# bruAristimunha/Synthetic-Sleep-EEG-Signal-Generation-using-Latent-Diffusion-Models

Hardware: AMD Instinct MI355X
Metric: EEG windows/sec (LDM train step) (higher is better)
Workload: dtype bf16; 1 GPU; LDM train step on raw (B,1,3072) windows: frozen AutoencoderKL[32,32,64] encode+sample x scale, add_noise, config_ldm.yaml UNet (30.5M params, latent_channels=1) fwd+bwd, epsilon MSE, Adam lr 1e-4 [BASELINE configs[2]/[3]: per-GPU batch 256 = global 2048 / 8]; per_gpu_batch=256, global_batch=256, latent_len=768, parallelism=dp1

## Files before the change

### synthetic-sleep-eeg-signal-generation-using-latent-diffusion-models_amd/csrc/norm.hip

```cpp
#include "common.h"
#include "internal.h"
#include <stdlib.h>

namespace {

constexpr int NT = 256;
constexpr int MAXG_LDS = 1024;
constexpr int GN_NSLOT = 64;
constexpr int GN_FOLD_MAX = 96;
constexpr size_t GN_REGION_FLOATS = (size_t)GN_NSLOT * 2 * 1024;
constexpr size_t GN_SLOT_OFFSET = 1u << 20;
constexpr size_t GN_SLOT_OFFSET_B = (1u << 20) + (512u << 10);
constexpr size_t GN_SLOT_OFFSET_C[2] = {24u << 20, (24u << 20) + (512u << 10)};
static inline size_t gn_slot_region(int region) { return region == 0 ? GN_SLOT_OFFSET_B : GN_SLOT_OFFSET_C[(region - 1) & 1]; }

template <typename T, int V> struct Vec;
template <> struct Vec<float, 4> { typedef float4 type; };
template <> struct Vec<bf16_t, 4> { typedef uint2 type; };
template <> struct Vec<f16_t, 4> { typedef uint2 type; };

template <typename T> __device__ __forceinline__ void load4(const T* p, float v[4]);
template <> __device__ __forceinline__ void load4<float>(const float* p, float v[4]) {
  float4 t = *(const float4*)p; v[0] = t.x; v[1] = t.y; v[2] = t.z; v[3] = t.w;
}
template <> __device__ __forceinline__ void load4<bf16_t>(const bf16_t* p, float v[4]) {
  uint2 t = *(const uint2*)p;
  v[0] = __uint_as_float(t.x << 16); v[1] = __uint_as_float(t.x & 0xffff0000u);
  v[2] = __uint_as_float(t.y << 16); v[3] = __uint_as_float(t.y & 0xffff0000u);
}
template <> __device__ __forceinline__ void load4<f16_t>(const f16_t* p, float v[4]) {
  uint2 t = *(const uint2*)p;
  v[0] = w16_lo<f16_t>(t.x); v[1] = w16_hi<f16_t>(t.x); v[2] = w16_lo<f16_t>(t.y); v[3] = w16_hi<f16_t>(t.y);
}
template <typename T> __device__ __forceinline__ void unpack4(const typename Vec<T, 4>::type& t, float v[4]);
template <> __device__ __forceinline__ void unpack4<f16_t>(const uint2& t, float v[4]) {
  v[0] = w16_lo<f16_t>(t.x); v[1] = w16_hi<f16_t>(t.x); v[2] = w16_lo<f16_t>(t.y); v[3] = w16_hi<f16_t>(t.y);
}
template <> __device__ __forceinline__ void unpack4<float>(const float4& t, float v[4]) { v[0] = t.x; v[1] = t.y; v[2] = t.z; v[3] = t.w; }
template <> __device__ __forceinline__ void unpack4<bf16_t>(const uint2& t, float v[4]) {
  v[0] = __uint_as_float(t.x << 16); v[1] = __uint_as_float(t.x & 0xffff0000u);
  v[2] = __uint_as_float(t.y << 16); v[3] = __uint_as_float(t.y & 0xffff0000u);
}
template <typename T> __device__ __forceinline__ void store4(T* p, const float v[4]);
template <> __device__ __forceinline__ void store4<float>(float* p, const float v[4]) {
  *(float4*)p = make_float4(v[0], v[1], v[2], v[3]);
}
template <> __device__ __forceinline__ void store4<bf16_t>(bf16_t* p, const float v[4]) {
  uint2 t;
  t.x = pack_bf16x2(v[0], v[1]);
  t.y = pack_bf16x2(v[2], v[3]);
  *(uint2*)p = t;
}
template <> __device__ __forceinline__ void store4<f16_t>(f16_t* p, const float v[4]) {
  uint2 t; t.x = pack_f16x2(v[0], v[1]); t.y = pack_f16x2(v[2], v[3]); *(uint2*)p = t;
}
template <typename T, int V> __device__ __forceinline__ void loadv(const T* p, float v[V]) {
  if constexpr (V == 4) load4<T>(p, v); else v[0] = ld_f32(p);
}
template <typename T, int V> __device__ __forceinline__ void storev(T* p, const float v[V]) {
  if constexpr (V == 4) store4<T>(p, v); else st_f32(p, v[0]);
}

template <typename T> __device__ __forceinline__ double gn_inv_n(int cpg, int L) {
  if constexpr (sizeof(T) == 2) return 1.0 / ((double)cpg * (double)L);
  else return (double)(1.0f / ((float)cpg * (float)L));
}
template <typename T> __device__ __forceinline__ float gn_split_group_mean(double sum, double inv_n) {
  if constexpr (sizeof(T) == 2) return (float)(sum * inv_n);
  else return (float)sum * (float)inv_n;
}

struct ColMap { int TX, TY, ncols; };
__device__ __forceinline__ ColMap colmap(int C, int V) {
  ColMap m; m.ncols = C / V;
  if (m.ncols >= NT) { m.TX = NT; m.TY = 1; } else { m.TX = m.ncols; m.TY = NT / m.ncols; }
  return m;
}

template <typename T, int V>
__global__ __launch_bounds__(NT) void gn_stats_kernel(const T* __restrict__ x, long ldx, double* __restrict__ sums,
                                                      int L, int C, int G, int rows_per_block) {
  __shared__ double acc[2 * MAXG_LDS];
  const int b = blockIdx.y, tid = threadIdx.x;
  const int cpg = C / G;
  for (int i = tid; i < 2 * G; i += NT) acc[i] = 0.0;
// ... 186 lines not shown
template <typename T, int V, int RS>
__global__ __launch_bounds__(NT) void gn_bwd_apply_kernel(const T* __restrict__ x, long ldx, const float* __restrict__ gamma,
                                                          const float* __restrict__ beta, const float* __restrict__ stats,
                                                          const T* __restrict__ dy, long lddy, const double* __restrict__ gsums,
                                                          T* __restrict__ dx, long lddx, const T* __restrict__ dxr, long lddxr,
                                                          int L, int C, int G, int silu, int rows_per_block) {
  const int b = blockIdx.y, tid = threadIdx.x, cpg = C / G;
  const ColMap cm = colmap(C, V);
  if (tid >= cm.TX * cm.TY) return;
  const int tx = tid % cm.TX, ty = tid / cm.TX;
  const double inv_n = gn_inv_n<T>(cpg, L);
  const int l0 = blockIdx.x * rows_per_block, l1 = min(L, l0 + rows_per_block);
  for (int col = tx; col < cm.ncols; col += cm.TX) {
    const int c = col * V, g = c / cpg;
    const float mean = stats[((long)b * G + g) * 2], rstd = stats[((long)b * G + g) * 2 + 1];
    const float m1 = gn_split_group_mean<T>(gsums[((long)b * G + g) * 2], inv_n), m2 = gn_split_group_mean<T>(gsums[((long)b * G + g) * 2 + 1], inv_n);
    float ga[V], be[V];
#pragma unroll
    for (int k = 0; k < V; k++) { ga[k] = gamma[c + k]; be[k] = beta[c + k]; }
#pragma unroll 2
    for (int l = l0 + ty; l < l1; l += cm.TY) {
      const long row = (long)b * L + l;
      float v[V], d[V], o[V];
      loadv<T, V>(x + row * ldx + c, v);
      load_dy_eff_c<T, V, RS>(dy, lddy, b, l, L, c, d);
#pragma unroll
      for (int k = 0; k < V; k++) {
        const float xh = (v[k] - mean) * rstd;
        float dz = d[k];
        if (silu) dz *= silu_grad_f(ga[k] * xh + be[k]);
        o[k] = rstd * (dz * ga[k] - m1 - xh * m2);
      }
      if (dxr) {
        float e[V];
        load_dy_eff_c<T, V, RS>(dxr, lddxr, b, l, L, c, e);
#pragma unroll
        for (int k = 0; k < V; k++) o[k] += e[k];
      }
      storev<T, V>(dx + row * lddx + c, o);
    }
  }
}

template <typename T>
__device__ __forceinline__ void load_dy_eff32(const char* base, unsigned ldb, unsigned cb, int l, int resample, float d[4]) {
  if (resample == 0) {
    load4<T>((const T*)(base + ((unsigned)l * ldb + cb)), d);
  } else if (resample == 1) {
    load4<T>((const T*)(base + ((unsigned)(l >> 1) * ldb + cb)), d);
#pragma unroll
    for (int k = 0; k < 4; k++) d[k] *= 0.5f;
  } else {
    float e[4];
    load4<T>((const T*)(base + ((unsigned)(2 * l) * ldb + cb)), d);
    load4<T>((const T*)(base + ((unsigned)(2 * l + 1) * ldb + cb)), e);
#pragma unroll
    for (int k = 0; k < 4; k++) d[k] += e[k];
  }
}
__device__ __forceinline__ long dy_rows(int L, int resample) { return resample == 1 ? L / 2 : (resample == 2 ? 2L * L : L); }

constexpr int NTB = 1024;
constexpr int RES_MAXG = 64;
constexpr int RES_MAXC = 256;

struct ResMap { int TX, TY, tx, ty, c, gl, b; bool act; };
template <int NTH>
__device__ __forceinline__ ResMap resmap(int CC, int C, int cpg, int xcd) {
  ResMap m; m.TX = CC / 4; m.TY = NTH / m.TX;
  const int tid = threadIdx.x;
  const int nchunk = C / CC, lin = blockIdx.x;
  int chunk, b;
  if (xcd) { const int x = lin & 7, j = lin >> 3; b = (j / nchunk) * 8 + x; chunk = j % nchunk; }
  else { chunk = lin % nchunk; b = lin / nchunk; }
  m.b = b;
  m.tx = tid % m.TX; m.ty = tid / m.TX;
  m.c = chunk * CC + m.tx * 4; m.gl = (m.tx * 4) / cpg;
  m.act = tid < m.TX * m.TY && m.c < C;
  return m;
}
__device__ __forceinline__ int res_row(int k, int ty, int TY, bool pair) {
  return pair ? 2 * ((k >> 1) * TY + ty) + (k & 1) : k * TY + ty;
}

#ifdef EEG_STAGE_TIMING
__device__ unsigned long long gn_tlog[4096 * 8];
#define GN_TSTAMP(k) do { if (threadIdx.x == 0) { asm volatile("s_waitcnt vmcnt(0) lgkmcnt(0)" ::: "memory"); gn_tlog[((size_t)blockIdx.y * gridDim.x + blockIdx.x) % 4096 * 8 + (k)] = __builtin_readcyclecounter(); } } while (0)
#else
#define GN_TSTAMP(k) do {} while (0)
#endif
template <typename T, int RPT, int NTH>
__global__ __launch_bounds__(NTH) void gn_fwd_resident_kernel(const T* __restrict__ x, long ldx, const float* __restrict__ gamma,
                                                              const float* __restrict__ beta, T* __restrict__ y, long ldy,
                                                              T* __restrict__ xr, long ldxr, float* __restrict__ stats,
                                                              int L, int C, int G, float eps, int silu, int resample, int CC, int xcd) {
  __shared__ double red[2 * RES_MAXG];
  GN_TSTAMP(0);
  const int cpg = C / G;
  const ResMap m = resmap<NTH>(CC, C, cpg, xcd);
  const int b = m.b;
  const bool pair = resample == 1;
  for (int i = threadIdx.x; i < 2 * RES_MAXG; i += NTH) red[i] = 0.0;
  typename Vec<T, 4>::type raw[RPT];
  const T* xb = x + (long)b * L * ldx + m.c;
  float pv = 0.f;
  if constexpr (sizeof(T) == 2) { if (m.act) pv = ld_f32<T>(x + (long)b * L * ldx + (m.c / cpg) * cpg); }
  if (m.act) {
#pragma unroll
    for (int k = 0; k < RPT; k++) {
      const int l = res_row(k, m.ty, m.TY, pair);
      if (l < L) raw[k] = *(const typename Vec<T, 4>::type*)(xb + (long)l * ldx);
    }
  }
  GN_TSTAMP(1);
  __syncthreads();
  GN_TSTAMP(2);
  const double inv_n = gn_inv_n<T>(cpg, L);
  float mean = 0.f, rstd = 0.f;
  if constexpr (sizeof(T) == 2) {
    float s1 = 0.f, s2 = 0.f;
    if (m.act) {
#pragma unroll
      for (int k = 0; k < RPT; k++) {
        if (res_row(k, m.ty, m.TY, pair) < L) {
          float v[4]; unpack4<T>(raw[k], v);
#pragma unroll
          for (int j = 0; j < 4; j++) v[j] -= pv;
          s1 += (v[0] + v[1]) + (v[2] + v[3]);
          s2 = fmaf(v[0], v[0], s2); s2 = fmaf(v[1], v[1], s2); s2 = fmaf(v[2], v[2], s2); s2 = fmaf(v[3], v[3], s2);
        }
      }
      atomicAdd(&red[m.gl], (double)s1); atomicAdd(&red[RES_MAXG + m.gl], (double)s2);
    }
    __syncthreads();
    GN_TSTAMP(3);
    GN_TSTAMP(4);
    if (!m.act) return;
    const double md = red[m.gl] * inv_n;
    double var = red[RES_MAXG + m.gl] * inv_n - md * md; if (var < 0.0) var = 0.0;
    mean = (float)((double)pv + md);
    rstd = rsqrtf((float)var + eps);
  } else {
  float s = 0.f;
  if (m.act) {
#pragma unroll
    for (int k = 0; k < RPT; k++) {
      if (res_row(k, m.ty, m.TY, pair) < L) { float v[4]; unpack4<T>(raw[k], v); s += (v[0] + v[1]) + (v[2] + v[3]); }
    }
    atomicAdd(&red[m.gl], (double)s);
  }
  __syncthreads();
  GN_TSTAMP(3);
  if (m.act) {
    mean = (float)(red[m.gl] * inv_n);
    float q = 0.f;
#pragma unroll
    for (int k = 0; k < RPT; k++) {
      if (res_row(k, m.ty, m.TY, pair) < L) {
        float v[4]; unpack4<T>(raw[k], v);
#pragma unroll
        for (int j = 0; j < 4; j++) { const float d = v[j] - mean; q += d * d; }
      }
    }
    atomicAdd(&red[RES_MAXG + m.gl], (double)q);
  }
  __syncthreads();
// ... 164 lines not shown
      const unsigned ldb = (unsigned)lddxr * (unsigned)sizeof(T);
#pragma unroll
      for (int k = 0; k < RPT; k++) { const int l = k * m.TY + m.ty, lc = l < L ? l : L - 1; er[k] = *(const typename Vec<T, 4>::type*)(q + ((unsigned)lc * ldb + cb)); }
    }
  }
  __syncthreads();
#ifdef EEG_GN_BWD_NO_LDS_ATOMICS
  if (m.act && m.ty == 0 && (m.tx * 4) % cpg == 0) {
    double p1 = 0.0, p2 = 0.0;
    for (int i = 0; i < cpg; i++) { const double g = (double)gamma[m.c + i]; p1 += g * redc[RES_MAXC + m.tx * 4 + i]; p2 += g * redc[m.tx * 4 + i]; }
    redg[2 * m.gl] = p1; redg[2 * m.gl + 1] = p2;
  }
#else
  if (m.act && m.ty == 0) {
    double p1 = 0.0, p2 = 0.0;
#pragma unroll
    for (int j = 0; j < 4; j++) { p1 += (double)ga[j] * redc[RES_MAXC + m.tx * 4 + j]; p2 += (double)ga[j] * redc[m.tx * 4 + j]; }
    atomicAdd(&redg[2 * m.gl], p1); atomicAdd(&redg[2 * m.gl + 1], p2);
  }
#endif
  GN_TSTAMP(3);
  __syncthreads();
  GN_TSTAMP(4);
  if (m.act) {
    const double inv_n = gn_inv_n<T>(cpg, L);
    const float m1 = (float)(redg[2 * m.gl] * inv_n), m2 = (float)(redg[2 * m.gl + 1] * inv_n);
    if (slots && m.ty == 0) {
      float* sl = slots + (size_t)(b % nslot) * 2 * C;
#pragma unroll
      for (int j = 0; j < 4; j++) { atomicAdd(&sl[m.c + j], (float)redc[m.tx * 4 + j]); atomicAdd(&sl[C + m.c + j], (float)redc[RES_MAXC + m.tx * 4 + j]); }
    }
    const float rm1 = rstd * m1, rm2 = rstd * m2;
    float gr[4];
#pragma unroll
    for (int j = 0; j < 4; j++) gr[j] = ga[j] * rstd;
    float cs[4] = {0.f, 0.f, 0.f, 0.f};
    char* dxs = (char*)(dx + (long)b * L * lddx);
    const char* dxrs = dxr ? (const char*)(dxr + (long)b * dy_rows(L, resample) * lddxr) : nullptr;
    const unsigned lddxb = (unsigned)lddx * (unsigned)sizeof(T), lddxrb = (unsigned)lddxr * (unsigned)sizeof(T);
    const char* dxr2s = dxr2 ? (const char*)(dxr2 + (long)b * L * lddxr2) : nullptr;
    const unsigned lddxr2b = (unsigned)lddxr2 * (unsigned)sizeof(T);
#pragma unroll
    for (int k = 0; k < RPT; k++) {
      const int l = k * m.TY + m.ty;
      if (l < L) {
        float v[4], o[4]; unpack4<T>(raw[k], v);
#pragma unroll
        for (int j = 0; j < 4; j++) {
          const float xh = fmaf(v[j], rstd, -mean * rstd);
          o[j] = fmaf(d[k][j], gr[j], fmaf(xh, -rm2, -rm1));
        }
        if (dxr) {
          float e[4];
          if constexpr (RAW0) unpack4<T>(er[k], e); else load_dy_eff32<T>(dxrs, lddxrb, cb, l, resample, e);
#pragma unroll
          for (int j = 0; j < 4; j++) o[j] += e[j];
        }
        if (dxr2) {
          float e[4];
          load4<T>((const T*)(dxr2s + ((unsigned)l * lddxr2b + cb)), e);
#pragma unroll
          for (int j = 0; j < 4; j++) o[j] += e[j];
        }
#pragma unroll
        for (int j = 0; j < 4; j++) cs[j] += o[j];
        store4<T>((T*)(dxs + ((unsigned)l * lddxb + cb)), o);
      }
    }
    if (colsum_ps) {
#pragma unroll
      for (int j = 0; j < 4; j++) atomicAdd(&redc[2 * RES_MAXC + m.tx * 4 + j], (double)cs[j]);
    }
  }
  GN_TSTAMP(5);
  if (colsum_ps) {
    __syncthreads();
    if (m.act && m.ty == 0) {
#pragma unroll
      for (int j = 0; j < 4; j++) colsum_ps[(long)b * ldps + m.c + j] = (float)redc[2 * RES_MAXC + m.tx * 4 + j];
    }
  }
}

constexpr int PIPE_RPT = 6;
constexpr int PIPE_SLAB = PIPE_RPT * NTB * 8;
constexpr int PIPE_OFF_ST = 3 * PIPE_SLAB;
constexpr int PIPE_OFF_RED = PIPE_OFF_ST + 1024;
constexpr int PIPE_LDS = PIPE_OFF_RED + (2 * RES_MAXG + 3 * RES_MAXC) * 8;

__device__ __forceinline__ void pipe_dma(const void* base, unsigned voff, unsigned lds_off) {
  const unsigned long long u = (unsigned long long)base;
  const unsigned lo = __builtin_amdgcn_readfirstlane((unsigned)u), hi = __builtin_amdgcn_readfirstlane((unsigned)(u >> 32));
  const unsigned long long b = ((unsigned long long)hi << 32) | lo;
  asm volatile("s_mov_b32 m0, %0\n\ts_nop 0\n\tglobal_load_lds_dwordx4 %1, %2" ::"s"(__builtin_amdgcn_readfirstlane(lds_off)), "v"(voff), "s"(b) : "memory", "m0");
}
#define PIPE_BARRIER() asm volatile("s_waitcnt lgkmcnt(0)\n\ts_barrier" ::: "memory")
#ifdef EEG_STAGE_TIMING
#define PIPE_TSTAMP(k, i) do { if (threadIdx.x == 0 && (k) < 8) gn_tlog[(size_t)(blockIdx.x % 512) * 64 + (k) * 8 + (i)] = __builtin_readcyclecounter(); } while (0)
#else
#define PIPE_TSTAMP(k, i) do {} while (0)
#endif

template <bool SILU, bool HAS_ER, typename T16 = bf16_t>
__global__ __launch_bounds__(NTB) void gn_bwd_pipe_kernel(const bf16_t* __restrict__ x, long ldx, const float* __restrict__ gamma,
                                                          const float* __restrict__ beta, const float* __restrict__ stats,
                                                          const bf16_t* __restrict__ dy, long lddy, bf16_t* __restrict__ dx, long lddx,
                                                          const bf16_t* __restrict__ dxr, long lddxr, float* __restrict__ slots,
                                                          float* __restrict__ colsum_ps, long ldps, int B, int L, int C, int G, int CC, int ndg) {
  extern __shared__ __attribute__((aligned(16))) char psm[];
  typedef __attribute__((address_space(3))) void* lds_ptr_t;
  double* const redg = (double*)(psm + PIPE_OFF_RED);
  double* const redc = redg + 2 * RES_MAXG;
  const int tid = threadIdx.x, lane = tid & 63;
  const unsigned wave_u = __builtin_amdgcn_readfirstlane((unsigned)(tid >> 6));
  const unsigned lds0 = (unsigned)(size_t)(lds_ptr_t)psm;
  const int cpg = C / G, nchunk = C / CC;
  const int TX = CC >> 2, TY = NTB / TX;
  const int tx = tid % TX, ty = tid / TX;
  const int xc = blockIdx.x & 7, mb = blockIdx.x >> 3, MB = gridDim.x >> 3;
  const int chunk = mb % nchunk, slot = mb / nchunk, nslot = MB / nchunk;
  const int c = chunk * CC + tx * 4, gl = (tx * 4) / cpg;
  const int noct = B >> 3;
  const int nk = slot < noct ? (noct - slot + nslot - 1) / nslot : 0;
  float ga[4], gl2[4], bl2[4];
#pragma unroll
  for (int j = 0; j < 4; j++) { ga[j] = gamma[c + j]; gl2[j] = ga[j] * 1.4426950408889634f; bl2[j] = beta[c + j] * 1.4426950408889634f; }
  for (int i = tid; i < 2 * RES_MAXG + 3 * RES_MAXC; i += NTB) redg[i] = 0.0;
  asm volatile("" :: "v"(ga[0]), "v"(ga[1]), "v"(ga[2]), "v"(ga[3]), "v"(bl2[0]), "v"(bl2[1]), "v"(bl2[2]), "v"(bl2[3]));
  const int LPR = CC >> 3;
  const int drow = (int)(wave_u * 64 + lane) / LPR, dcol = lane % LPR;
  const unsigned vx = (unsigned)drow * (unsigned)ldx * 2u + (unsigned)dcol * 16u, sx = (unsigned)(1024 / LPR) * (unsigned)ldx * 2u;
  const unsigned vd = (unsigned)drow * (unsigned)lddy * 2u + (unsigned)dcol * 16u, sd = (unsigned)(1024 / LPR) * (unsigned)lddy * 2u;
  const unsigned ve = (unsigned)drow * (unsigned)lddxr * 2u + (unsigned)dcol * 16u, se = (unsigned)(1024 / LPR) * (unsigned)lddxr * 2u;
  const unsigned st_bytes = (unsigned)B * (unsigned)G * 8u;
  const unsigned st_sub = ((unsigned)(chunk * (CC / cpg)) * 8u) & 15u;
  auto issue_xd = [&](int b) __attribute__((always_inline)) {
    const char* xs = (const char*)(x + (long)b * L * ldx + chunk * CC);
    const char* ds = (const char*)(dy + (long)b * L * lddy + chunk * CC);
#pragma unroll
    for (int i = 0; i < 3; i++) pipe_dma(xs, vx + i * sx, lds0 + (unsigned)(i * 16 + wave_u) * 1024u);
#pragma unroll
    for (int i = 0; i < 3; i++) pipe_dma(ds, vd + i * sd, lds0 + PIPE_SLAB + (unsigned)(i * 16 + wave_u) * 1024u);
    {
      const unsigned a0 = (((unsigned)b * (unsigned)G + (unsigned)(chunk * (CC / cpg))) * 8u) & ~15u;
      unsigned a = a0 + (unsigned)lane * 16u; if (a > st_bytes - 16u) a = st_bytes - 16u;
      pipe_dma(stats, a, lds0 + PIPE_OFF_ST);
    }
  };
  auto issue_e = [&](int b) __attribute__((always_inline)) {
    const char* es = (const char*)(dxr + (long)b * L * lddxr + chunk * CC);
#pragma unroll
    for (int i = 0; i < 3; i++) pipe_dma(es, ve + i * se, lds0 + 2 * PIPE_SLAB + (unsigned)(i * 16 + wave_u) * 1024u);
  };
  if (nk > 0) { issue_xd(slot * 8 + xc); if constexpr (HAS_ER) issue_e(slot * 8 + xc); }
  const double inv_n = gn_inv_n<T16>(cpg, L);
  const unsigned rowb = (unsigned)CC * 2u;
  const unsigned lrd0 = (unsigned)ty * rowb + (unsigned)tx * 8u, lrds = (unsigned)TY * rowb;
  const unsigned lddxb = (unsigned)lddx * 2u;
  const unsigned st0 = (unsigned)ty * lddxb + (unsigned)c * 2u, sts = (unsigned)TY * lddxb;
  asm volatile("s_waitcnt vmcnt(0)" ::: "memory");
  for (int k = 0; k < nk; k++) {
    const int b = (slot + k * nslot) * 8 + xc;
    PIPE_TSTAMP(k, 0);
    PIPE_BARRIER();
    PIPE_TSTAMP(k, 1);
    uint2 raw[PIPE_RPT], dr[PIPE_RPT];
// ... 36 lines not shown
      double p1 = 0.0, p2 = 0.0;
#pragma unroll
      for (int j = 0; j < 4; j++) { p1 += (double)ga[j] * redc[RES_MAXC + tx * 4 + j]; p2 += (double)ga[j] * redc[tx * 4 + j]; }
      atomicAdd(&redg[2 * gl], p1); atomicAdd(&redg[2 * gl + 1], p2);
    }
    if constexpr (HAS_ER) {
      if (k + 1 < nk) asm volatile("s_waitcnt vmcnt(7)" ::: "memory"); else asm volatile("s_waitcnt vmcnt(0)" ::: "memory");
    }
    PIPE_BARRIER();
    PIPE_TSTAMP(k, 5);
    {
      const float m1 = (float)(redg[2 * gl] * inv_n), m2 = (float)(redg[2 * gl + 1] * inv_n);
      if (slots && ty == 0) {
        float* sl = slots + (size_t)(b % ndg) * 2 * C;
#pragma unroll
        for (int j = 0; j < 4; j++) { atomicAdd(&sl[c + j], (float)redc[tx * 4 + j]); atomicAdd(&sl[C + c + j], (float)redc[RES_MAXC + tx * 4 + j]); }
      }
      const float rm1 = rstd * m1, rm2 = rstd * m2;
      const float a2 = -rm2 * rstd, b2 = fmaf(-rm2, nmr, -rm1);
      float gr[4];
#pragma unroll
      for (int j = 0; j < 4; j++) gr[j] = ga[j] * rstd;
      float cs[4] = {0.f, 0.f, 0.f, 0.f};
      char* dxs = (char*)(dx + (long)b * L * lddx);
#pragma unroll
      for (int r = 0; r < PIPE_RPT; r++) {
        float v[4], o[4]; unpack4<T16>(raw[r], v);
#pragma unroll
        for (int j = 0; j < 4; j++) o[j] = fmaf(d[r][j], gr[j], fmaf(v[j], a2, b2));
        if constexpr (HAS_ER) {
          float e[4]; unpack4<T16>(*(const uint2*)(psm + 2 * PIPE_SLAB + lrd0 + (unsigned)r * lrds), e);
#pragma unroll
          for (int j = 0; j < 4; j++) o[j] += e[j];
        }
        if (colsum_ps) {
#pragma unroll
          for (int j = 0; j < 4; j++) cs[j] += o[j];
        }
        store4<T16>((T16*)(dxs + (st0 + (unsigned)r * sts)), o);
      }
      if (colsum_ps) {
#pragma unroll
        for (int j = 0; j < 4; j++) atomicAdd(&redc[2 * RES_MAXC + tx * 4 + j], (double)cs[j]);
      }
    }
    PIPE_TSTAMP(k, 6);
    PIPE_BARRIER();
    if (ty == 0) {
#pragma unroll
      for (int j = 0; j < 4; j++) {
        if (colsum_ps) colsum_ps[(long)b * ldps + c + j] = (float)redc[2 * RES_MAXC + tx * 4 + j];
        redc[tx * 4 + j] = 0.0; redc[RES_MAXC + tx * 4 + j] = 0.0; redc[2 * RES_MAXC + tx * 4 + j] = 0.0;
      }
    }
    if (tid < 2 * RES_MAXG) redg[tid] = 0.0;
    if (k + 1 < nk) {
      if constexpr (HAS_ER) { issue_e((slot + (k + 1) * nslot) * 8 + xc); asm volatile("s_waitcnt vmcnt(9)" ::: "memory"); }
      else asm volatile("s_waitcnt vmcnt(6)" ::: "memory");
    }
    PIPE_TSTAMP(k, 7);
  }
}


struct GnRoute { int family, vec, nth, rpt, cc, xcd; };
static thread_local GnRoute g_gn_route[2] = {{0, 0, 0, 0, 0, 0}, {0, 0, 0, 0, 0, 0}};
inline void gn_note(int bwd, int family, int vec, int nth, int rpt, int cc, int xcd) { g_gn_route[bwd] = GnRoute{family, vec, nth, rpt, cc, xcd}; }

int resident_chunk(int L, int C, int G, int resample_pair, int rpt_max, int* rpt_out, int nth = NTB) {
  const int cpg = C / G;
  if (C % 4 != 0 || cpg % 4 != 0) return 0;
  int best = 0, best_rpt = 0;
  for (int mlt = 1; mlt * cpg <= RES_MAXC && mlt <= RES_MAXG; mlt++) {
    const int cc = mlt * cpg;
    if (C % cc != 0) continue;
    const int tx = cc / 4, ty = nth / tx;
    if (ty < 1) break;
    int rpt = resample_pair ? 2 * ((L / 2 + ty - 1) / ty) : (L + ty - 1) / ty;
    if (rpt > rpt_max) break;
    best = cc; best_rpt = rpt;
  }
  *rpt_out = best_rpt;
  return best;
}

int grid_for(long total_threads, eegldm_ctx* ctx) {
  long blocks = (total_threads + NT - 1) / NT;
  long cap = (long)ctx->num_cu * 16;
  return (int)(blocks < cap ? (blocks < 1 ? 1 : blocks) : cap);
}

int pick_lsplit(int B, int L, int C, eegldm_ctx* ctx, int* rows_per_block, int per_cu = 8, int min_rows = 16) {
  int want = (ctx->num_cu * per_cu + B - 1) / B;
  int maxsplit = (L + min_rows - 1) / min_rows;
  int ls = want < 1 ? 1 : (want > maxsplit ? maxsplit : want);
  int rpb = (L + ls - 1) / ls;
  *rows_per_block = rpb;
  return (L + rpb - 1) / rpb;
}

template <typename T, int V>
int gn_fwd_t(eegldm_ctx* ctx, const void* x, long ldx, const float* gamma, const float* beta, void* y, long ldy,
             float* stats, int B, int L, int C, int G, float eps, int silu, int resample, void* xr, long ldxr) {
  if constexpr (V == 4) {
    EEG_ENV_VAR(bool, off, getenv("EEGLDM_GN_NO_RESIDENT") != nullptr);
    constexpr int fwd_rpt_max = 12;
    EEG_ENV_VAR(int, fwd_nth, getenv("EEGLDM_GN_FWD_NTH") ? atoi(getenv("EEGLDM_GN_FWD_NTH")) : 1024);
    int nth = (fwd_nth == 512 || fwd_nth == 256) ? fwd_nth : 1024;
    int rpt = 0; int cc = off ? 0 : resident_chunk(L, C, G, resample == 1, fwd_rpt_max, &rpt, nth);
    EEG_ENV_VAR(bool, no_few, getenv("EEGLDM_GN_NO_FEW_SLAB_NARROW") != nullptr);
    if (!no_few && cc && nth == 1024 && (long)(C / cc) * B <= ctx->num_cu / 4) {
      int rpt2 = 0; const int cc2 = resident_chunk(L, C, G, resample == 1, fwd_rpt_max, &rpt2, 256);
      if (cc2 && cc2 * (int)sizeof(T) >= 32) { nth = 256; cc = cc2; rpt = rpt2; }
    }
    constexpr long fwd_bpc = 4;
    constexpr bool no_xcd = false;
    constexpr int narrow_min = 32;
    const bool can_xcd = !no_xcd && B % 8 == 0;
    const int min_row = nth == 1024 ? (can_xcd ? narrow_min : 128) : 32;
    if (cc && (cc * (int)sizeof(T) < min_row || (long)(C / cc) * B > fwd_bpc * ctx->num_cu * (1024 / nth))) cc = 0;
    if (cc) {
      const int xcd = ((nth < 1024 || cc * (int)sizeof(T) < 128) && can_xcd) ? 1 : 0;
      const dim3 grid((unsigned)((long)(C / cc) * B));
#define GN_FWD_RES1(R, N) hipLaunchKernelGGL((gn_fwd_resident_kernel<T, R, N>), grid, dim3(N), 0, ctx->stream, (const T*)x, ldx, gamma, beta, \
                                         (T*)y, ldy, (T*)xr, ldxr, stats, L, C, G, eps, silu, resample, cc, xcd)
#define GN_FWD_RES(R) do { if (nth == 1024) GN_FWD_RES1(R, 1024); else if (nth == 512) GN_FWD_RES1(R, 512); else GN_FWD_RES1(R, 256); } while (0)
      gn_note(0, 2, 1, nth, rpt <= 6 ? 6 : 12, cc, xcd);
      if (rpt <= 6) GN_FWD_RES(6); else GN_FWD_RES(12);
#undef GN_FWD_RES
#undef GN_FWD_RES1
      LAUNCH_CHECK();
      return 0;
    }
  }
  double* sums = (double*)ctx->scratch;
  int rpb; int ls = pick_lsplit(B, L, C, ctx, &rpb);
  gn_note(0, 1, V == 4, NT, 0, 0, 0);
  hipLaunchKernelGGL((gn_stats_kernel<T, V>), dim3(ls, B), dim3(NT), 0, ctx->stream, (const T*)x, ldx, sums, L, C, G, rpb);
  LAUNCH_CHECK();
  hipLaunchKernelGGL(gn_finalize_kernel, dim3((B * G + 255) / 256), dim3(256), 0, ctx->stream, sums, stats, B * G,
                     (double)(C / G) * (double)L, eps);
  LAUNCH_CHECK();
  int rpb2; int ls2 = pick_lsplit(B, resample == 1 ? L / 2 : L, C, ctx, &rpb2, 16, 8);
  hipLaunchKernelGGL((gn_apply_kernel<T, V>), dim3(ls2, B), dim3(NT), 0, ctx->stream, (const T*)x, ldx, gamma,
                     beta, stats, (T*)y, ldy, (T*)xr, ldxr, L, C, G, silu, resample, rpb2);
  LAUNCH_CHECK();
  return 0;
}

template <typename T, int V>
int gn_bwd_t(eegldm_ctx* ctx, const void* x, long ldx, const float* gamma, const float* beta, const float* stats,
             const void* dy, long lddy, void* dx, long lddx, float* dgamma, float* dbeta, int B, int L, int C, int G,
             int silu, int resample, const void* dxr, long lddxr, float* colsum_ps, long ldps, int* colsum_done,
             const void* dxr2, long lddxr2, int* dxr2_done, int* slots_deferred, int defer_region) {
  if (colsum_done) *colsum_done = 0;
  if (dxr2_done) *dxr2_done = 0;
  if (slots_deferred) *slots_deferred = 0;
  if (!dxr2_done || lddxr2 % 4 != 0) dxr2 = nullptr;
  if constexpr (V == 4) {
    EEG_ENV_VAR(bool, off, getenv("EEGLDM_GN_NO_RESIDENT") != nullptr);
    EEG_ENV_VAR(int, bwd_nth, getenv("EEGLDM_GN_BWD_NTH") ? atoi(getenv("EEGLDM_GN_BWD_NTH")) : 1024);
    EEG_ENV_VAR(bool, unfenced, getenv("EEGLDM_GN_NARROW_UNFENCED") != nullptr);
#ifdef EEG_GN_NO_FENCE
    const int nth = (bwd_nth == 512 || bwd_nth == 256) ? bwd_nth : 1024;
#else
    const int nth = ((bwd_nth == 512 || bwd_nth == 256) && (unfenced || (!ctx->side_on && g_eeg_live_ctx <= 1))) ? bwd_nth : 1024;
// ... 22 lines not shown
          if (dgamma) slots = (float*)((char*)ctx->scratch + (defer ? gn_slot_region(defer_region) : GN_SLOT_OFFSET));
          if (det) {
            ndg = B;
            EEG_TRY(eeg_det_buffer(ctx, (size_t)ndg * 2 * C * sizeof(float), &slots));
            HIP_TRY(hipMemsetAsync(slots, 0, (size_t)ndg * 2 * C * sizeof(float), ctx->stream));
          }
          constexpr bool no_batch_p = false;
          const bool batched = defer && ctx->defer_wgrad && !no_batch_p && C <= 1024 && ctx->gn_fold_count < GN_FOLD_MAX;
          if (batched) {
            if (!ctx->gn_slot_arena) {
              HIP_TRY(hipMalloc(&ctx->gn_slot_arena, (size_t)GN_FOLD_MAX * GN_REGION_FLOATS * sizeof(float)));
              HIP_TRY(hipMemsetAsync(ctx->gn_slot_arena, 0, (size_t)GN_FOLD_MAX * GN_REGION_FLOATS * sizeof(float), ctx->stream));
            }
            slots = ctx->gn_slot_arena + (size_t)ctx->gn_fold_count * GN_REGION_FLOATS;
            ctx->gn_fold_pending.push_back({slots, dgamma, dbeta, C});
            ctx->gn_fold_count++;
          }
          static DevOnce attr_once;
          if (attr_once.need(ctx->device)) {
            HIP_TRY(hipFuncSetAttribute((const void*)gn_bwd_pipe_kernel<true, true, T>, hipFuncAttributeMaxDynamicSharedMemorySize, PIPE_LDS));
            HIP_TRY(hipFuncSetAttribute((const void*)gn_bwd_pipe_kernel<true, false, T>, hipFuncAttributeMaxDynamicSharedMemorySize, PIPE_LDS));
            HIP_TRY(hipFuncSetAttribute((const void*)gn_bwd_pipe_kernel<false, true, T>, hipFuncAttributeMaxDynamicSharedMemorySize, PIPE_LDS));
            HIP_TRY(hipFuncSetAttribute((const void*)gn_bwd_pipe_kernel<false, false, T>, hipFuncAttributeMaxDynamicSharedMemorySize, PIPE_LDS));
          }
          const dim3 grid((unsigned)(8 * nslot * nchunk));
          gn_note(1, 3, 1, NTB, PIPE_RPT, pcc, 1);
#define GN_BWD_PIPE(SL, ER) hipLaunchKernelGGL((gn_bwd_pipe_kernel<SL, ER, T>), grid, dim3(NTB), PIPE_LDS, ctx->stream, (const bf16_t*)x, ldx, gamma, beta, stats, \
                                           (const bf16_t*)dy, lddy, (bf16_t*)dx, lddx, (const bf16_t*)dxr, lddxr, slots, colsum_ps, ldps, B, L, C, G, pcc, ndg)
          if (silu) { if (dxr) GN_BWD_PIPE(true, true); else GN_BWD_PIPE(true, false); }
          else { if (dxr) GN_BWD_PIPE(false, true); else GN_BWD_PIPE(false, false); }
#undef GN_BWD_PIPE
          LAUNCH_CHECK();
          if (det) {
            EEG_TRY(ew_fold_partials_det(ctx, slots, ndg, 2 * C, 0, C, dgamma)); EEG_TRY(ew_fold_partials_det(ctx, slots, ndg, 2 * C, C, C, dbeta));
          } else if (slots && !defer) {
            hipLaunchKernelGGL(gn_slot_reduce_kernel, dim3((2 * C + 255) / 256), dim3(256), 0, ctx->stream, slots, dgamma, dbeta, C, (double*)ctx->scratch, 0, ndg);
            LAUNCH_CHECK();
          }
          if (defer) *slots_deferred = batched ? 2 : 1;
          if (colsum_done && colsum_ps) *colsum_done = 1;
          return 0;
        }
      }
    }
    int rpt = 0; int cc = off ? 0 : resident_chunk(L, C, G, 0, sizeof(T) == 2 ? 12 : 8, &rpt, nth);
    constexpr long bwd_bpc = 8;
    constexpr int bwd_minrow = 128, narrow_min = 32;
    constexpr bool no_xcd = false;
    const bool can_xcd = !no_xcd && B % 8 == 0;
    const int min_row = nth == 1024 ? (can_xcd && narrow_min < bwd_minrow ? narrow_min : bwd_minrow) : 32;
    if (cc && (cc * (int)sizeof(T) < min_row || (long)(C / cc) * B > bwd_bpc * ctx->num_cu * (1024 / nth))) cc = 0;
    if (cc) {
      const int xcd = ((nth < 1024 || cc * (int)sizeof(T) < 128) && can_xcd) ? 1 : 0;
      const dim3 grid((unsigned)((long)(C / cc) * B));
      constexpr bool no_defer = false;
      const bool det = eeg_deterministic() && dgamma;
      const bool defer = slots_deferred && dgamma && !no_defer && !det;
      float* slots = dgamma ? (float*)((char*)ctx->scratch + (defer ? gn_slot_region(defer_region) : GN_SLOT_OFFSET)) : nullptr;
      int nslot = GN_NSLOT;
      if (det) {
        nslot = B;
        EEG_TRY(eeg_det_buffer(ctx, (size_t)nslot * 2 * C * sizeof(float), &slots));
        HIP_TRY(hipMemsetAsync(slots, 0, (size_t)nslot * 2 * C * sizeof(float), ctx->stream));
      }
      constexpr bool no_batch = false;
      const bool batched = defer && ctx->defer_wgrad && !no_batch && C <= 1024 && ctx->gn_fold_count < GN_FOLD_MAX;
      if (batched) {
        if (!ctx->gn_slot_arena) {
          HIP_TRY(hipMalloc(&ctx->gn_slot_arena, (size_t)GN_FOLD_MAX * GN_REGION_FLOATS * sizeof(float)));
          HIP_TRY(hipMemsetAsync(ctx->gn_slot_arena, 0, (size_t)GN_FOLD_MAX * GN_REGION_FLOATS * sizeof(float), ctx->stream));
        }
        slots = ctx->gn_slot_arena + (size_t)ctx->gn_fold_count * GN_REGION_FLOATS;
        ctx->gn_fold_pending.push_back({slots, dgamma, dbeta, C});
        ctx->gn_fold_count++;
      }
#define GN_BWD_RES3(R, RAW, SL, N) hipLaunchKernelGGL((gn_bwd_resident_kernel<T, R, RAW, SL, N>), grid, dim3(N), 0, ctx->stream, (const T*)x, ldx, gamma, beta, stats, \
                                         (const T*)dy, lddy, (T*)dx, lddx, (const T*)dxr, lddxr, slots, colsum_ps, ldps, L, C, G, silu, resample, cc, (const T*)dxr2, lddxr2, xcd, nslot)
#define GN_BWD_RES2(R, RAW, SL) do { if (nth == 1024) GN_BWD_RES3(R, RAW, SL, 1024); else if (nth == 512) GN_BWD_RES3(R, RAW, SL, 512); else GN_BWD_RES3(R, RAW, SL, 256); } while (0)
      constexpr bool raw0 = true;
#define GN_BWD_RES1(R, RAW) do { if (silu) GN_BWD_RES2(R, RAW, true); else GN_BWD_RES2(R, RAW, false); } while (0)
#define GN_BWD_RES(R) do { if (resample == 0 && raw0) GN_BWD_RES1(R, true); else GN_BWD_RES1(R, false); } while (0)
      constexpr int RLO = sizeof(T) == 2 ? 6 : 4, RHI = sizeof(T) == 2 ? 12 : 8;
      gn_note(1, 2, 1, nth, rpt <= RLO ? RLO : RHI, cc, xcd);
      if (rpt <= RLO) GN_BWD_RES(RLO); else GN_BWD_RES(RHI);
#undef GN_BWD_RES
#undef GN_BWD_RES1
#undef GN_BWD_RES2
#undef GN_BWD_RES3
      LAUNCH_CHECK();
      if (det) {
        EEG_TRY(ew_fold_partials_det(ctx, slots, nslot, 2 * C, 0, C, dgamma)); EEG_TRY(ew_fold_partials_det(ctx, slots, nslot, 2 * C, C, C, dbeta));
      } else if (slots && !defer) {
        hipLaunchKernelGGL(gn_slot_reduce_kernel, dim3((2 * C + 255) / 256), dim3(256), 0, ctx->stream, slots, dgamma, dbeta, C, (double*)ctx->scratch, 0, nslot);
        LAUNCH_CHECK();
      }
      if (defer) *slots_deferred = batched ? 2 : 1;
      if (colsum_done && colsum_ps) *colsum_done = 1;
      if (dxr2) *dxr2_done = 1;
      return 0;
    }
  }
  double* gsums = (double*)ctx->scratch;
  int rpb; int ls = pick_lsplit(B, L, C, ctx, &rpb);
  gn_note(1, 1, V == 4, NT, 0, 0, 0);
  float* slots = dgamma ? (float*)((char*)ctx->scratch + GN_SLOT_OFFSET) : nullptr;
  int nslot = GN_NSLOT;
  if (slots && eeg_deterministic()) {
    nslot = ls * B;
    EEG_TRY(eeg_det_buffer(ctx, (size_t)nslot * 2 * C * sizeof(float), &slots));
    HIP_TRY(hipMemsetAsync(slots, 0, (size_t)nslot * 2 * C * sizeof(float), ctx->stream));
  }
#define GN_BWD_SPLIT(RS) do { \
    hipLaunchKernelGGL((gn_bwd_reduce_kernel<T, V, RS>), dim3(ls, B), dim3(NT), 0, ctx->stream, (const T*)x, ldx, gamma, beta, stats, \
                       (const T*)dy, lddy, gsums, slots, L, C, G, silu, rpb, nslot); \
    hipLaunchKernelGGL((gn_bwd_apply_kernel<T, V, RS>), dim3(ls2, B), dim3(NT), 0, ctx->stream, (const T*)x, ldx, gamma, \
                       beta, stats, (const T*)dy, lddy, gsums, (T*)dx, lddx, (const T*)dxr, lddxr, L, C, G, silu, rpb2); } while (0)
  int rpb2; int ls2 = pick_lsplit(B, L, C, ctx, &rpb2, 16, 8);
  if (resample == 0) GN_BWD_SPLIT(0); else if (resample == 1) GN_BWD_SPLIT(1); else GN_BWD_SPLIT(2);
#undef GN_BWD_SPLIT
  LAUNCH_CHECK();
  const int n_gs = 2 * B * G;
  hipLaunchKernelGGL(gn_slot_reduce_kernel, dim3(((2 * C > n_gs ? 2 * C : n_gs) + 255) / 256), dim3(256), 0, ctx->stream, slots, dgamma, dbeta, C, gsums, n_gs, nslot);
  LAUNCH_CHECK();
  return 0;
}

constexpr int FLAT_NT = 256;
template <typename T> struct Chunk8;
template <> struct Chunk8<bf16_t> {
  typedef uint4 raw_t;
  static __device__ __forceinline__ raw_t load(const bf16_t* p) { return *(const uint4*)p; }
  static __device__ __forceinline__ void unpack(const raw_t& r, float v[8]) {
    v[0] = __uint_as_float(r.x << 16); v[1] = __uint_as_float(r.x & 0xffff0000u); v[2] = __uint_as_float(r.y << 16); v[3] = __uint_as_float(r.y & 0xffff0000u);
    v[4] = __uint_as_float(r.z << 16); v[5] = __uint_as_float(r.z & 0xffff0000u); v[6] = __uint_as_float(r.w << 16); v[7] = __uint_as_float(r.w & 0xffff0000u);
  }
  static __device__ __forceinline__ void touch(raw_t& r) { asm volatile("" : "+v"(r.x), "+v"(r.y), "+v"(r.z), "+v"(r.w)); }
  static __device__ __forceinline__ void store(bf16_t* p, const float v[8]) {
    uint4 t; t.x = pack_bf16x2(v[0], v[1]); t.y = pack_bf16x2(v[2], v[3]); t.z = pack_bf16x2(v[4], v[5]); t.w = pack_bf16x2(v[6], v[7]);
    *(uint4*)p = t;
  }
};
template <> struct Chunk8<f16_t> {
  typedef uint4 raw_t;
  static __device__ __forceinline__ raw_t load(const f16_t* p) { return *(const uint4*)p; }
  static __device__ __forceinline__ void unpack(const raw_t& r, float v[8]) {
    v[0] = w16_lo<f16_t>(r.x); v[1] = w16_hi<f16_t>(r.x); v[2] = w16_lo<f16_t>(r.y); v[3] = w16_hi<f16_t>(r.y);
    v[4] = w16_lo<f16_t>(r.z); v[5] = w16_hi<f16_t>(r.z); v[6] = w16_lo<f16_t>(r.w); v[7] = w16_hi<f16_t>(r.w);
  }
  static __device__ __forceinline__ void touch(raw_t& r) { asm volatile("" : "+v"(r.x), "+v"(r.y), "+v"(r.z), "+v"(r.w)); }
  static __device__ __forceinline__ void store(f16_t* p, const float v[8]) {
    uint4 t; t.x = pack_f16x2(v[0], v[1]); t.y = pack_f16x2(v[2], v[3]); t.z = pack_f16x2(v[4], v[5]); t.w = pack_f16x2(v[6], v[7]);
    *(uint4*)p = t;
  }
};
template <> struct Chunk8<float> {
  struct raw_t { float4 a, b; };
  static __device__ __forceinline__ raw_t load(const float* p) { raw_t r; r.a = *(const float4*)p; r.b = *(const float4*)(p + 4); return r; }
  static __device__ __forceinline__ void unpack(const raw_t& r, float v[8]) {
    v[0] = r.a.x; v[1] = r.a.y; v[2] = r.a.z; v[3] = r.a.w; v[4] = r.b.x; v[5] = r.b.y; v[6] = r.b.z; v[7] = r.b.w;
  }
  static __device__ __forceinline__ void touch(raw_t&) {}
  static __device__ __forceinline__ void store(float* p, const float v[8]) {
    *(float4*)p = make_float4(v[0], v[1], v[2], v[3]); *(float4*)(p + 4) = make_float4(v[4], v[5], v[6], v[7]);
  }
};
template <int K, int NW = 4> __device__ __forceinline__ void flat_block_sum(float (&v)[K], float* sm) {
#pragma unroll
// ... 405 lines not shown
```

Before: 14460 windows/s.

## Add specialized full-slab resident GroupNorm backward kernel with compile-time flags

Adds a new GroupNorm backward resident kernel used when the row slab exactly covers L. Options such as residual inputs, colsum, SiLU and resample mode become template parameters dispatched through a static switch over 96 variants. The kernel issues all x and dy loads up front, batches residual loads, and drops runtime bounds and flag checks. The aim is to cut branching and address arithmetic and to overlap memory latency. The cost is many more kernel instantiations and higher register pressure from holding rows in registers.

New measurement: 14710 windows/s, median of 6. +1.7%, better.

```diff
diff --git a/synthetic-sleep-eeg-signal-generation-using-latent-diffusion-models_amd/csrc/norm.hip b/synthetic-sleep-eeg-signal-generation-using-latent-diffusion-models_amd/csrc/norm.hip
--- a/synthetic-sleep-eeg-signal-generation-using-latent-diffusion-models_amd/csrc/norm.hip
+++ b/synthetic-sleep-eeg-signal-generation-using-latent-diffusion-models_amd/csrc/norm.hip
@@ -1,6 +1,7 @@
 #include "common.h"
 #include "internal.h"
 #include <stdlib.h>
+#include <type_traits>
 
 namespace {
 
@@ -353,6 +354,9 @@
 __device__ __forceinline__ int res_row(int k, int ty, int TY, bool pair) {
   return pair ? 2 * ((k >> 1) * TY + ty) + (k & 1) : k * TY + ty;
 }
+__device__ __forceinline__ void gn_issue_order() { asm volatile("" ::: "memory"); }
+__device__ __forceinline__ void keep_packed(uint2& r) { asm volatile("" : "+v"(r.x), "+v"(r.y)); }
+__device__ __forceinline__ void keep_packed(float4& r) { asm volatile("" : "+v"(r.x), "+v"(r.y), "+v"(r.z), "+v"(r.w)); }
 
 #ifdef EEG_STAGE_TIMING
 __device__ unsigned long long gn_tlog[4096 * 8];
@@ -683,6 +687,154 @@
   }
 }
 
+template <typename T, int RS> struct GnDyRow {
+  unsigned stride, off;
+  __device__ __forceinline__ GnDyRow(int ty, int TY, unsigned ldb, unsigned cb) {
+    stride = (RS == 0 ? (unsigned)TY : RS == 1 ? (unsigned)TY >> 1 : 2u * (unsigned)TY) * ldb;
+    off = (RS == 0 ? (unsigned)ty : RS == 1 ? (unsigned)ty >> 1 : 2u * (unsigned)ty) * ldb + cb;
+  }
+  __device__ __forceinline__ typename Vec<T, 4>::type ld(const char* base, int k, unsigned second) const {
+    return *(const typename Vec<T, 4>::type*)(base + (size_t)k * stride + (off + second));
+  }
+};
+template <typename T, int RS>
+__device__ __forceinline__ void gn_dy_eff(const typename Vec<T, 4>::type& a, const typename Vec<T, 4>::type& a2, float d[4]) {
+  unpack4<T>(a, d);
+  if constexpr (RS == 1) {
+#pragma unroll
+    for (int j = 0; j < 4; j++) d[j] *= 0.5f;
+  } else if constexpr (RS == 2) {
+    float e[4]; unpack4<T>(a2, e);
+#pragma unroll
+    for (int j = 0; j < 4; j++) d[j] += e[j];
+  }
+}
+template <typename T, int RPT, int RS, bool SILU, int FL>
+__global__ __launch_bounds__(NTB) void gn_bwd_resident_full_kernel(const T* __restrict__ x, long ldx, const float* __restrict__ gamma,
+                                                                   const float* __restrict__ beta, const float* __restrict__ stats,
+                                                                   const T* __restrict__ dy, long lddy, T* __restrict__ dx, long lddx,
+                                                                   const T* __restrict__ dxr, long lddxr, float* __restrict__ slots,
+                                                                   float* __restrict__ colsum_ps, long ldps, int L, int C, int G, int CC,
+                                                                   const T* __restrict__ dxr2, long lddxr2, int xcd, int nslot) {
+  typedef typename Vec<T, 4>::type V4;
+  constexpr bool HAS_DXR = (FL & 1) != 0, HAS_DXR2 = (FL & 2) != 0, HAS_CS = (FL & 4) != 0;
+  constexpr int NDY = RS == 2 ? 2 : 1;
+  __shared__ double redg[2 * RES_MAXG];
+  __shared__ double redc[3 * RES_MAXC];
+  const int cpg = C / G;
+  const ResMap m = resmap<NTB>(CC, C, cpg, xcd);
+  const int b = m.b;
+  const float* st = stats + ((long)b * G + m.c / cpg) * 2;
+  const float mean = st[0], rstd = st[1];
+  float ga[4], be[4];
+#pragma unroll
+  for (int j = 0; j < 4; j++) { ga[j] = gamma[m.c + j]; be[j] = beta[m.c + j]; }
+  gn_issue_order();
+  V4 raw[RPT], dr[NDY * RPT];
+  float d[RPT][4];
+  const unsigned cb = (unsigned)m.c * (unsigned)sizeof(T);
+  const unsigned ldxb = (unsigned)ldx * (unsigned)sizeof(T), lddyb = (unsigned)lddy * (unsigned)sizeof(T);
+  const char* xs = (const char*)(x + (long)b * L * ldx);
+  const char* dys = (const char*)(dy + (long)b * dy_rows(L, RS) * lddy);
+  const GnDyRow<T, 0> rx(m.ty, m.TY, ldxb, cb);
+  const GnDyRow<T, RS> rdy(m.ty, m.TY, lddyb, cb);
+#pragma unroll
+  for (int k = 0; k < RPT; k++) {
+    raw[k] = rx.ld(xs, k, 0);
+    dr[NDY * k] = rdy.ld(dys, k, 0);
+    if constexpr (RS == 2) dr[2 * k + 1] = rdy.ld(dys, k, lddyb);
+    gn_issue_order();
+  }
+  for (int i = threadIdx.x; i < 2 * RES_MAXG + 3 * RES_MAXC; i += NTB) { if (i < 2 * RES_MAXG) redg[i] = 0.0; else redc[i - 2 * RES_MAXG] = 0.0; }
+  __syncthreads();
+  {
+    float dg[4] = {0.f, 0.f, 0.f, 0.f}, db[4] = {0.f, 0.f, 0.f, 0.f};
+    const float nmr = -mean * rstd;
+#pragma unroll
+    for (int k = 0; k < RPT; k++) {
+      float v[4]; unpack4<T>(raw[k], v);
+      gn_dy_eff<T, RS>(dr[NDY * k], dr[NDY * k + NDY - 1], d[k]);
+#pragma unroll
+      for (int j = 0; j < 4; j++) {
+        const float xh = fmaf(v[j], rstd, nmr);
+        float dz = d[k][j];
+        if constexpr (SILU) dz *= silu_grad_f(fmaf(ga[j], xh, be[j]));
+        d[k][j] = dz;
+        dg[j] = fmaf(dz, xh, dg[j]); db[j] += dz;
+      }
+    }
+#pragma unroll
+    for (int j = 0; j < 4; j++) { atomicAdd(&redc[m.tx * 4 + j], (double)dg[j]); atomicAdd(&redc[RES_MAXC + m.tx * 4 + j], (double)db[j]); }
+  }
+#pragma unroll
+  for (int k = 0; k < RPT; k++) keep_packed(raw[k]);
+  constexpr bool ER_BATCH = HAS_DXR && !HAS_DXR2 && RS != 2;
+  V4 er[ER_BATCH ? RPT : 1];
+  const char* dxrs = HAS_DXR ? (const char*)(dxr + (long)b * dy_rows(L, RS) * lddxr) : nullptr;
+  const unsigned lddxrb = (unsigned)lddxr * (unsigned)sizeof(T);
+  const GnDyRow<T, RS> rer(m.ty, m.TY, lddxrb, cb);
+  if constexpr (ER_BATCH) {
+#pragma unroll
+    for (int k = 0; k < RPT; k++) er[k] = rer.ld(dxrs, k, 0);
+  }
+  __syncthreads();
+  if (m.ty == 0) {
+    double p1 = 0.0, p2 = 0.0;
+#pragma unroll
+    for (int j = 0; j < 4; j++) { p1 += (double)ga[j] * redc[RES_MAXC + m.tx * 4 + j]; p2 += (double)ga[j] * redc[m.tx * 4 + j]; }
+    atomicAdd(&redg[2 * m.gl], p1); atomicAdd(&redg[2 * m.gl + 1], p2);
+  }
+  __syncthreads();
+  const double inv_n = gn_inv_n<T>(cpg, L);
+  const float m1 = (float)(redg[2 * m.gl] * inv_n), m2 = (float)(redg[2 * m.gl + 1] * inv_n);
+  if (slots && m.ty == 0) {
+    float* sl = slots + (size_t)(b % nslot) * 2 * C;
+#pragma unroll
+    for (int j = 0; j < 4; j++) { atomicAdd(&sl[m.c + j], (float)redc[m.tx * 4 + j]); atomicAdd(&sl[C + m.c + j], (float)redc[RES_MAXC + m.tx * 4 + j]); }
+  }
+  const float rm1 = rstd * m1, rm2 = rstd * m2;
+  float gr[4];
+#pragma unroll
+  for (int j = 0; j < 4; j++) gr[j] = ga[j] * rstd;
+  float cs[4] = {0.f, 0.f, 0.f, 0.f};
+  char* dxs = (char*)(dx + (long)b * L * lddx);
+  const char* dxr2s = HAS_DXR2 ? (const char*)(dxr2 + (long)b * L * lddxr2) : nullptr;
+  const GnDyRow<T, 0> rdx(m.ty, m.TY, (unsigned)lddx * (unsigned)sizeof(T), cb), rdx2(m.ty, m.TY, (unsigned)lddxr2 * (unsigned)sizeof(T), cb);
+#pragma unroll
+  for (int k = 0; k < RPT; k++) {
+    float v[4], o[4]; unpack4<T>(raw[k], v);
+#pragma unroll
+    for (int j = 0; j < 4; j++) {
+      const float xh = fmaf(v[j], rstd, -mean * rstd);
+      o[j] = fmaf(d[k][j], gr[j], fmaf(xh, -rm2, -rm1));
+    }
+    if constexpr (HAS_DXR) {
+      float e[4];
+      if constexpr (ER_BATCH) gn_dy_eff<T, RS>(er[k], er[k], e);
+      else gn_dy_eff<T, RS>(rer.ld(dxrs, k, 0), rer.ld(dxrs, k, lddxrb), e);
+#pragma unroll
+      for (int j = 0; j < 4; j++) o[j] += e[j];
+    }
+    if constexpr (HAS_DXR2) {
+      float e[4]; unpack4<T>(rdx2.ld(dxr2s, k, 0), e);
+#pragma unroll
+      for (int j = 0; j < 4; j++) o[j] += e[j];
+    }
+#pragma unroll
+    for (int j = 0; j < 4; j++) cs[j] += o[j];
+    store4<T>((T*)(dxs + (size_t)k * rdx.stride + rdx.off), o);
+  }
+  if constexpr (HAS_CS) {
+#pragma unroll
+    for (int j = 0; j < 4; j++) atomicAdd(&redc[2 * RES_MAXC + m.tx * 4 + j], (double)cs[j]);
+    __syncthreads();
+    if (m.ty == 0) {
+#pragma unroll
+      for (int j = 0; j < 4; j++) colsum_ps[(long)b * ldps + m.c + j] = (float)redc[2 * RES_MAXC + m.tx * 4 + j];
+    }
+  }
+}
+
 constexpr int PIPE_RPT = 6;
 constexpr int PIPE_SLAB = PIPE_RPT * NTB * 8;
 constexpr int PIPE_OFF_ST = 3 * PIPE_SLAB;
@@ -885,6 +1037,16 @@
   }
   *rpt_out = best_rpt;
   return best;
+}
+
+bool resident_full_slab(int L, int cc, int rpt_inst) {
+  const int tx = cc / 4;
+  return tx >= 1 && NTB % tx == 0 && (NTB / tx) % 2 == 0 && rpt_inst % 2 == 0 && (long)rpt_inst * (NTB / tx) == L;
+}
+
+template <int N, typename F> void gn_static_switch(int v, F&& f) {
+  if (v == N - 1) f(std::integral_constant<int, N - 1>());
+  else if constexpr (N > 1) gn_static_switch<N - 1>(v, f);
 }
 
 int grid_for(long total_threads, eegldm_ctx* ctx) {
@@ -1073,7 +1235,16 @@
 #define GN_BWD_RES(R) do { if (resample == 0 && raw0) GN_BWD_RES1(R, true); else GN_BWD_RES1(R, false); } while (0)
       constexpr int RLO = sizeof(T) == 2 ? 6 : 4, RHI = sizeof(T) == 2 ? 12 : 8;
       gn_note(1, 2, 1, nth, rpt <= RLO ? RLO : RHI, cc, xcd);
-      if (rpt <= RLO) GN_BWD_RES(RLO); else GN_BWD_RES(RHI);
+      EEG_ENV_VAR(bool, no_stream, getenv("EEGLDM_GN_NO_STREAM") != nullptr);
+      if (!no_stream && nth == NTB && resident_full_slab(L, cc, rpt <= RLO ? RLO : RHI)) {
+        const int sel = (dxr ? 1 : 0) | (dxr2 ? 2 : 0) | (colsum_ps ? 4 : 0) | (silu ? 8 : 0) | (rpt <= RLO ? 0 : 16) | ((resample == 1 ? 1 : resample == 2 ? 2 : 0) << 5);
+        gn_static_switch<96>(sel, [&](auto s) {
+          constexpr int S = decltype(s)::value;
+          hipLaunchKernelGGL((gn_bwd_resident_full_kernel<T, (S & 16) ? RHI : RLO, (S / 32), (S & 8) != 0, (S & 7)>), grid, dim3(NTB), 0, ctx->stream,
+                             (const T*)x, ldx, gamma, beta, stats, (const T*)dy, lddy, (T*)dx, lddx, (const T*)dxr, lddxr, slots, colsum_ps, ldps,
+                             L, C, G, cc, (const T*)dxr2, lddxr2, xcd, nslot);
+        });
+      } else if (rpt <= RLO) GN_BWD_RES(RLO); else GN_BWD_RES(RHI);
 #undef GN_BWD_RES
 #undef GN_BWD_RES1
 #undef GN_BWD_RES2
```
